# pculbertson/argus

Measured on AMD Instinct MI355X. Metric: train images/sec + val SE(3) geodesic err, 2x256x256 RGB, higher is better.
Workload: dtype bf16; 1 GPU; configs[1] cube_unity_data_small-shaped: fused train step, 64 samples (128 images) of 256x256 per rank, 2 cams, ResNet-50 + MLP head, bf16; batch_per_rank=64, global_batch=64, parallelism=dp1

## Files before the change

### argus_amd/csrc/conv.hip

```cpp
#include "common.h"
#include "internal.h"
#include "ktimer.h"
#include "igemm.h"
#include "lds_dma.h"

namespace argus {

template <typename T>
ARGUS_DEV u32x4 bn_relu_chunk(u32x4 v, const float* __restrict__ sc, const float* __restrict__ sh, int ch) {
  constexpr int E = Chunk<T>::E;
  float f[E];
  unpack(v, f);
#pragma unroll
  for (int j = 0; j < E; ++j) f[j] = fmaxf(fmaf(f[j], sc[ch + j], sh[ch + j]), 0.f);
  return pack(f);
}

constexpr int kProLds = 512;

template <typename T> struct ProCoef {
  float s[Chunk<T>::E], h[Chunk<T>::E];
  ARGUS_DEV void load(const float* __restrict__ sc, const float* __restrict__ sh, int ch) {
#pragma unroll
    for (int j = 0; j < Chunk<T>::E; j += 4) {
// ... 1599 lines not shown
  return dgrad_stages_prologue(d, p.f8 ? ARGUS_BF16 : dtype, p) ? 1 : 0;
}

static int dgrad_bn_impl(const argus_conv_desc& d, int dtype, const void* dy, const void* wt, void* dm,
                         const void* addend, const argus_bn_bwd_epilogue* bn, const argus_bn_bwd_prologue* pro,
                         bool x8, hipStream_t st) {
  if (int e = check_desc(d)) return e;
  const bool f8 = dtype == ARGUS_FP8;
  if (f8) dtype = ARGUS_BF16;
  if (d.stem) { set_error("conv_dgrad_bn: the stem input has no gradient"); return ARGUS_ERR_ARG; }
  static const argus_bn_bwd_epilogue no_epilogue = {};
  const bool epi = bn != nullptr;
  if (!epi) bn = &no_epilogue;
  const bool yrec = epi && bn->y_x;
  if (yrec && (dtype != ARGUS_BF16 || bn->y || !bn->y_w || bn->mask_mode != 3 || bn->y_k <= 0 || bn->y_k % 64)) {
    set_error("conv_dgrad_bn: y recompute needs bf16, mask mode 3, y == NULL, y_w and y_k % 64 == 0");
    return ARGUS_ERR_ARG;
  }
  if ((epi && ((!bn->y && !yrec) || !bn->mean || !bn->invstd || !bn->part || (bn->mask_mode != 2 && bn->mask_mode != 3))) ||
      (bn->mask_mode == 2 && (!bn->scale || !bn->shift || bn->y2)) || (bn->mask_mode == 3 && !bn->mask_bits) ||
      (bn->y2 && (!bn->mean2 || !bn->invstd2 || !bn->part2)) || (bn->y && bn->y == dm)) {
    set_error("conv_dgrad_bn: bad BN-backward epilogue arguments");
    return ARGUS_ERR_ARG;
  }
  if (pro && (!pro->y || !pro->ca || !pro->cb || !pro->cc || (pro->dy_out && (pro->dy_out == dy || pro->dy_out == dm)))) {
    set_error("conv_dgrad_bn: bad apply-prologue arguments");
    return ARGUS_ERR_ARG;
  }
  const Policy pol = policy_of(d);
  if (x8 && (pro || yrec || addend || (epi && bn->mask_mode != 2))) {
    set_error("conv_dgrad_bn_x8: no apply prologue, addend or y recompute; BN epilogue mask mode 2 only");
    return ARGUS_ERR_ARG;
  }
  if (!x8 && pol[kP1x1Dgrad] && epi && !yrec && bn->mask_mode == 3 && pro && !pro->dy_out && p1x1_ok(d, dtype) &&
      !(f8 && (pol[kFp8Passes] & 4)) && bn->workspace && bn->gamma && bn->ca && bn->cb && bn->cc &&
      (!bn->y2 || (bn->gamma2 && bn->ca2 && bn->cb2 && bn->cc2))) {
    dgrad_work(d, dtype, addend != nullptr, true, true, bn->y2 != nullptr);
    g_launch_bytes += 2.0 * d.n * d.ho * d.wo * d.k;
    return p1x1_launch(d, dy, wt, dm, addend, bn, pro, st);
  }
  IgParams p;
  dgrad_params(d, pol, dy, wt, dm, addend, nullptr, p);
  p.f8 = f8 && !yrec;
  if (x8) {
    int f8f, f8d;
    wp_f8_layouts(d, f8f, f8d);
    p.x8 = 1;
    p.bb.mode = epi ? 2 : 0;
    if (!f8d || !conv3x3_halo_x8_ok(p)) {
      set_error("conv_dgrad_bn_x8: not served (3x3 stride-1 halo shapes, K % 128, MX-fp8 dgrad weights: "
                "policy key 37 bit 2)");
      return ARGUS_ERR_ARG;
    }
    p.bb.mode = 0;
  }
  if (yrec) { p.bb.yx = bn->y_x; p.bb.yw = bn->y_w; p.bb.yk = bn->y_k; }
  if (pro) {
    if (!dgrad_stages_prologue(d, dtype, p)) {
      if (!pro->dy_out) {
        set_error("conv_dgrad_bn: this dgrad cannot stage the apply prologue; dy_out is required");
        return ARGUS_ERR_ARG;
      }
      if (int e = argus_bn_bwd_apply(dtype, (int64_t)d.n * d.ho * d.wo, d.k, dy, 0, nullptr, pro->y, nullptr,
                                     nullptr, pro->ca, pro->cb, pro->cc, pro->dy_out, nullptr, nullptr, nullptr,
                                     nullptr, nullptr, nullptr, st))
        return e;
      p.a = pro->dy_out;
    } else {
      p.ap.y = pro->y; p.ap.ca = pro->ca; p.ap.cb = pro->cb; p.ap.cc = pro->cc; p.ap.out = pro->dy_out;
    }
  }
// ... 301 lines not shown
```

### argus_amd/csrc/conv_p1x1.hip

```cpp
#include "common.h"
#include "igemm.h"
#include "internal.h"
#include "ktimer.h"

namespace argus {

namespace {
constexpr int kP1BM = 64, kP1BN = 128, kP1LDC = kP1BN + 8;

template <int KC> ARGUS_DEV int p1_pos(int row, int chunk) {
  return row * KC + (chunk ^ (KC >= 16 ? (row & 15) : ((row >> 1) & 7)));
}
}

struct P1Params {
  const bf16* dm;
  const bf16* ay;
  const float *ca, *cb, *cc;
  const bf16* wd;
  const bf16* addend;
  bf16* out;
  BnBwdEpi bb;
  BnFin fin;
  int P, N, G, NB, tiles;
};

template <int K, int BW>
__global__ __launch_bounds__(256, K >= 256 ? 1 : 2) void p1x1_dgrad_kernel(const P1Params p) {
  constexpr bool DUAL = BW == 4;
  constexpr int KC = K / 8;
  constexpr int ARP = 256 / KC;
  constexpr int APS = kP1BM / ARP;
  constexpr int W_B = kP1BN * K * 2, A_B = kP1BM * K * 2, C_B = kP1BM * kP1LDC * 2;
  constexpr int RED_B = 8 * 16 * 16 * 8;
  static_assert(C_B >= RED_B && A_B + C_B >= 256 * 32, "scratch");
  __shared__ __attribute__((aligned(16))) u32x4 lds[(W_B + A_B + C_B) / 16];
  __shared__ int fin_flag;
  u32x4* Wl = lds;
  u32x4* Al = lds + W_B / 16;
  bf16* Cs = reinterpret_cast<bf16*>(lds + (W_B + A_B) / 16);

  const int total = p.G * p.NB;
  const int wid = xcd_remap(blockIdx.x, total);
  const int nb = wid % p.NB, g0 = wid / p.NB;
  const int tid = threadIdx.x, lane = tid & 63, wave = tid >> 6;
  const int wm = wave >> 1, wn = wave & 1;
  const int g = lane >> 4, i16 = lane & 15;

#pragma unroll
  for (int i = 0; i < kP1BN * KC / 256; ++i) {
    const int idx = tid + 256 * i, r = idx / KC, c = idx - r * KC;
    Wl[p1_pos<KC>(r, c)] = ld16(p.wd + (size_t)(nb * kP1BN + r) * K + c * 8);
  }
  const int ac = tid % KC, ar0 = tid / KC;
  float ca[8], cb[8], cc[8];
  BwdEpiAcc<bf16, 3>::ld(ca, p.ca + ac * 8);
  BwdEpiAcc<bf16, 3>::ld(cb, p.cb + ac * 8);
  BwdEpiAcc<bf16, 3>::ld(cc, p.cc + ac * 8);
  const int ec = tid % 16, rg = tid / 16;
  const int col = nb * kP1BN + ec * 8;
  BwdEpiAcc<bf16, BW> bwd;
  bwd.init(p.bb, col);

  struct APre { u32x4 dm[APS], y[APS]; };
  struct EPre { u32x4 add[4], y[4], y2[DUAL ? 4 : 1]; unsigned bits[4]; };
  auto load_a = [&](int t, APre& S) {
#pragma unroll
    for (int i = 0; i < APS; ++i) {
      const int m = min(t * kP1BM + ar0 + ARP * i, p.P - 1);
      S.dm[i] = ld16(p.dm + (size_t)m * K + ac * 8);
      S.y[i] = ld16(p.ay + (size_t)m * K + ac * 8);
    }
  };
  auto load_e = [&](int t, EPre& S) {
#pragma unroll
    for (int i = 0; i < 4; ++i) {
      const size_t off = (size_t)min(t * kP1BM + rg + 16 * i, p.P - 1) * p.N + col;
      if (p.addend) S.add[i] = ld16(p.addend + off);
      S.y[i] = ld16(reinterpret_cast<const bf16*>(p.bb.y) + off);
      if constexpr (DUAL) S.y2[i] = ld16(reinterpret_cast<const bf16*>(p.bb.y2) + off);
      S.bits[i] = p.bb.bits[off / 8];
    }
  };

  APre A;
  EPre Ep;
  int t = g0;
  if (t < p.tiles) {
    load_a(t, A);
    load_e(t, Ep);
  }
  __syncthreads();
  for (; t < p.tiles; t += p.G) {
#pragma unroll
    for (int i = 0; i < APS; ++i) {
      const int r = ar0 + ARP * i;
      float d[8], yv[8];
      unpack(A.dm[i], d);
      unpack(A.y[i], yv);
#pragma unroll
      for (int j = 0; j < 8; ++j) d[j] = fmaf(ca[j], d[j], fmaf(cb[j], yv[j], cc[j]));
      Al[p1_pos<KC>(r, ac)] = sel(t * kP1BM + r < p.P, pack(d));
    }
    const int tn = t + p.G;
    if (tn < p.tiles) load_a(tn, A);
    __syncthreads();

    f32x4 acc[2][4];
#pragma unroll
    for (int mi = 0; mi < 2; ++mi)
#pragma unroll
      for (int ni = 0; ni < 4; ++ni) acc[mi][ni] = f32x4{0.f, 0.f, 0.f, 0.f};
#pragma unroll
    for (int kk = 0; kk < K / 32; ++kk) {
      const int ch = 4 * kk + g;
      u32x4 fa[2], fb[4];
#pragma unroll
      for (int mi = 0; mi < 2; ++mi) fa[mi] = Al[p1_pos<KC>(32 * wm + 16 * mi + i16, ch)];
#pragma unroll
      for (int ni = 0; ni < 4; ++ni) fb[ni] = Wl[p1_pos<KC>(64 * wn + 16 * ni + i16, ch)];
#pragma unroll
      for (int mi = 0; mi < 2; ++mi)
#pragma unroll
        for (int ni = 0; ni < 4; ++ni) Mma<bf16>::run(acc[mi][ni], fa[mi], fb[ni]);
    }
#pragma unroll
    for (int mi = 0; mi < 2; ++mi)
#pragma unroll
      for (int ni = 0; ni < 4; ++ni)
#pragma unroll
        for (int r = 0; r < 4; ++r)
          Cs[(32 * wm + 16 * mi + 4 * g + r) * kP1LDC + 64 * wn + 16 * ni + i16] = (bf16)acc[mi][ni][r];
    __syncthreads();

#pragma unroll
    for (int i = 0; i < 4; ++i) {
      const int r = rg + 16 * i;
      const int m = t * kP1BM + r;
      if (m >= p.P) continue;
      u32x4 v = *reinterpret_cast<const u32x4*>(Cs + r * kP1LDC + ec * 8);
      if (p.addend) {
        float f[8], o[8];
        unpack(v, f);
        unpack(Ep.add[i], o);
#pragma unroll
        for (int j = 0; j < 8; ++j) f[j] += o[j];
        v = pack(f);
      }
      st16_nt(p.out + (size_t)m * p.N + col, bwd.step(v, Ep.y[i], DUAL ? Ep.y2[DUAL ? i : 0] : Ep.y[i], Ep.bits[i]));
    }
    if (tn < p.tiles) load_e(tn, Ep);
  }
  __syncthreads();
  bwd.template reduce<kP1BN, 256>(p.bb, reinterpret_cast<float2*>(Cs), rg, 16, ec, (size_t)g0, p.N, nb * kP1BN);
  if (p.fin.mode) {
    __syncthreads();
    bn_fin_arrive<256, kP1BN>(p.fin, g0, nb, reinterpret_cast<double2*>(Al), &fin_flag);
  }
}


static int p1_occ(int K) { return K >= 256 ? 1 : 2; }

bool p1x1_ok(const argus_conv_desc& d, int dtype) {
  return dtype == ARGUS_BF16 && !d.stem && d.r == 1 && d.s == 1 && d.stride == 1 && d.pad == 0 &&
         (d.k == 64 || d.k == 128 || d.k == 256) && d.c % kP1BN == 0 && d.h == d.ho && d.w == d.wo &&
         (long)d.n * d.h * d.w > 0;
}

int p1x1_rows(const argus_conv_desc& d) {
  const int tiles = (int)(((long)d.n * d.h * d.w + kP1BM - 1) / kP1BM);
  const int nb = d.c / kP1BN;
  int G = p1_occ(d.k) * 256 / nb;
  if (G < 1) G = 1;
  return G < tiles ? G : tiles;
}

int p1x1_launch(const argus_conv_desc& d, const void* dm, const void* wd, void* out, const void* addend,
                const argus_bn_bwd_epilogue* bn, const argus_bn_bwd_prologue* pro, hipStream_t st) {
  P1Params p{};
  p.dm = reinterpret_cast<const bf16*>(dm);
  p.ay = reinterpret_cast<const bf16*>(pro->y);
  p.ca = pro->ca; p.cb = pro->cb; p.cc = pro->cc;
  p.wd = reinterpret_cast<const bf16*>(wd);
  p.addend = reinterpret_cast<const bf16*>(addend);
  p.out = reinterpret_cast<bf16*>(out);
  p.P = d.n * d.h * d.w;
  p.N = d.c;
  p.NB = d.c / kP1BN;
  p.tiles = (p.P + kP1BM - 1) / kP1BM;
  p.G = p1x1_rows(d);
  BnBwdEpi& b = p.bb;
  b.y = bn->y; b.mean = bn->mean; b.invstd = bn->invstd; b.bits = bn->mask_bits; b.y2 = bn->y2;
  b.mean2 = bn->mean2; b.invstd2 = bn->invstd2;
  b.part = reinterpret_cast<float2*>(bn->part); b.part2 = reinterpret_cast<float2*>(bn->part2);
  b.mode = 3; b.prow = p.G;
  if (bn->workspace) {
    BnFin& f = p.fin;
    f.mode = 2; f.C = d.c; f.count = (long long)p.P;
    f.cnt = reinterpret_cast<unsigned*>(bn->workspace);
    f.red = reinterpret_cast<double2*>(reinterpret_cast<char*>(bn->workspace) + kBnCounterBytes);
    f.part = reinterpret_cast<const float2*>(bn->part); f.part2 = reinterpret_cast<const float2*>(bn->part2);
    f.gamma = bn->gamma; f.bmean = bn->mean; f.binvstd = bn->invstd;
    f.dgamma = bn->dgamma; f.dbeta = bn->dbeta; f.ca = bn->ca; f.cb = bn->cb; f.cc = bn->cc;
    f.gamma2 = bn->gamma2; f.bmean2 = bn->mean2; f.binvstd2 = bn->invstd2;
    f.dgamma2 = bn->dgamma2; f.dbeta2 = bn->dbeta2; f.ca2 = bn->ca2; f.cb2 = bn->cb2; f.cc2 = bn->cc2;
    bn_fin_plan(f, p.G, 1);
    f.rows = f.T;
  }
  const dim3 grid(p.G * p.NB);
  const bool dual = bn->y2 != nullptr;
  static const char* names[3][2] = {{"argus::p1x1_dgrad_kernel<64, 3>", "argus::p1x1_dgrad_kernel<64, 4>"},
                                    {"argus::p1x1_dgrad_kernel<128, 3>", "argus::p1x1_dgrad_kernel<128, 4>"},
                                    {"argus::p1x1_dgrad_kernel<256, 3>", "argus::p1x1_dgrad_kernel<256, 4>"}};
  const int ki = d.k == 64 ? 0 : (d.k == 128 ? 1 : 2);
  const char* nm = names[ki][dual];
  if (d.k == 64) {
    if (dual) timed_launch(nm, p1x1_dgrad_kernel<64, 4>, grid, dim3(256), st, p);
    else timed_launch(nm, p1x1_dgrad_kernel<64, 3>, grid, dim3(256), st, p);
  } else if (d.k == 128) {
    if (dual) timed_launch(nm, p1x1_dgrad_kernel<128, 4>, grid, dim3(256), st, p);
    else timed_launch(nm, p1x1_dgrad_kernel<128, 3>, grid, dim3(256), st, p);
  } else {
    if (dual) timed_launch(nm, p1x1_dgrad_kernel<256, 4>, grid, dim3(256), st, p);
    else timed_launch(nm, p1x1_dgrad_kernel<256, 3>, grid, dim3(256), st, p);
  }
  return check_launch("p1x1_dgrad_kernel");
}

struct P1FParams {
  const bf16* x;
  const bf16* w;
  float2* part;
  int* counts;
  int P, N, G, NB, tiles;
  BnFwdFin ffin;
};

template <int K, int BNC>
__global__ __launch_bounds__(256) void p1x1_fwd_stats_kernel(const P1FParams p) {
  constexpr int KC = K / 8;
  constexpr int ARP = 256 / KC;
  constexpr int APS = kP1BM / ARP;
  constexpr int NI = BNC / 32;
  constexpr int DEPTH = K <= 256 ? 2 : 1;
  constexpr int W_B = BNC * K * 2, A_B = kP1BM * K * 2;
  static_assert(A_B >= 2 * BNC * 16, "reduction scratch");
  __shared__ __attribute__((aligned(16))) u32x4 lds[(W_B + A_B) / 16];
  u32x4* Wl = lds;
  u32x4* Al = lds + W_B / 16;

  const int total = p.G * p.NB;
  const int wid = xcd_remap(blockIdx.x, total);
  const int nb = wid % p.NB, g0 = wid / p.NB;
  const int tid = threadIdx.x, lane = tid & 63, wave = tid >> 6;
  const int wm = wave >> 1, wn = wave & 1;
  const int g = lane >> 4, i16 = lane & 15;

// ... 205 lines not shown
```

### argus_amd/engine.py

```python
from __future__ import annotations

import ctypes as C
import contextlib
from dataclasses import dataclass

import torch

from argus_amd._lib import BnFwdFin, BF16, F32, FP8, BnBwdEpilogue, BnBwdPrologue, ConvDesc, lib, ptr, stream


@dataclass(frozen=True)
class Block:
    prefix: str
    cin: int
    width: int
    cout: int
    stride: int
    has_ds: bool


def resnet50_blocks() -> list[Block]:
    blocks, inplanes = [], 64
    for L, (planes, n, stride) in enumerate([(64, 3, 1), (128, 4, 2), (256, 6, 2), (512, 3, 2)], start=1):
        for i in range(n):
# ... 35 lines not shown
        self.rdim = resnet_output_dim
        self.dtype = dtype
        low = dtype in ("bf16", "fp8")
        self.dt = BF16 if low else F32
        self.cdt = FP8 if dtype == "fp8" else self.dt
        self.tdt = torch.bfloat16 if low else torch.float32
        self.E = 8 if low else 4
        self.materialize = low
        self.device = torch.device(device)
        self.blocks = resnet50_blocks()
        self.shape = None
        self.saved = False
        self.debug: dict | None = None
        self.wgrad_overlap = True
        self.fuse_apply = True
        self.wgrad_apply = True
        self.fold_fin = True
        self.fold_fwd_fin = False
        self.fold_stem_fin = True
        self._side: torch.cuda.Stream | None = None
        self._pending: dict = {}
        self._last_side = None
        self.side_batch = True
        self._deferred: list = []
        self._side_seq = 0
        self._waited_seq = 0
        self._stem_overlap = True
        self.tail_main = True
        self._tail: list = []
        self.dy_ring = 12
        self.side_priority = 0
        self.fuse_dgw = True
        self.fuse_out = True
        self.yrec_epi = False
        self.y3_free = False
        self.x8 = True
        self.a2_in_stats = False

    def _t(self, *shape, dtype=None):
        return torch.empty(shape, dtype=dtype or self.tdt, device=self.device)

    def _f(self, *shape):
        return torch.empty(shape, dtype=torch.float32, device=self.device)

    def ensure(self, B: int, H: int, W: int) -> None:
        if self.shape == (B, H, W):
            return
        self.shape = (B, H, W)
        N = B * self.n_cams
        self.N = N
        L = self.L
        dt = self.dt
        convs: dict[str, _Conv] = {}

        def add(name, n, h, w, c, k, ks, s, p, stem=False):
            d = ConvDesc(n, h, w, c, k, ks, ks, s, p, _out(h, ks, s, p), _out(w, ks, s, p), int(stem)).with_tuning(
                self.tuning)
            if stem:
                wf = self._t(k, 256)
                wd = None
            else:
                wf = self._t(k, ks * ks * c)
                wd = self._t(c, ks * ks * k)
            rows = L.dll.argus_conv_fwd_stat_rows(C.byref(d), self.cdt)
            tile = L.dll.argus_conv_fwd_stat_tile(C.byref(d), dt)
            fl = C.c_int64(0)
            tags = tuple(L.dll.argus_conv_launch_info(C.byref(d), dt, ps, C.byref(fl)) for ps in range(3))
            so = (L.dll.argus_conv_fwd_stats_only_rows(C.byref(d), BF16),
                  L.dll.argus_conv_fwd_stats_only_tile(C.byref(d), BF16))
            pb = max(L.dll.argus_conv_fwd_stat_part_bytes(C.byref(d), self.cdt, 0),
                     L.dll.argus_conv_fwd_stat_part_bytes(C.byref(d), dt, 0),
                     L.dll.argus_conv_fwd_stat_part_bytes(C.byref(d), BF16, 1))
            convs[name] = _Conv(name, d, wf, wd, rows, tile, tags, fl.value, *so, part_bytes=pb)
            return d.ho, d.wo

        H1, W1 = add("resnet.conv1", N, H, W, 3, 64, 7, 2, 3, stem=True)
        H2, W2 = _out(H1, 3, 2, 1), _out(W1, 3, 2, 1)
        self.stem_hw = (H1, W1)
        self.pool_hw = (H2, W2)
        self.x0 = self._t(N, H, W, 4)
        self.y0 = self._t(N, H1, W1, 64)
        self.p0 = self._t(N, H2, W2, 64)
        self.amax = torch.empty((N, H2, W2, 64), dtype=torch.uint8, device=self.device)
        act = []
        h, w = H2, W2
        max_elems = N * H1 * W1 * 64
        for b in self.blocks:
            add(b.prefix + ".conv1", N, h, w, b.cin, b.width, 1, 1, 0)
            ho, wo = add(b.prefix + ".conv2", N, h, w, b.width, b.width, 3, b.stride, 1)
            add(b.prefix + ".conv3", N, ho, wo, b.width, b.cout, 1, 1, 0)
            if b.has_ds:
                add(b.prefix + ".downsample.0", N, h, w, b.cin, b.cout, 1, b.stride, 0)
            a = {
                "hw_in": (h, w), "hw": (ho, wo),
                "y1": self._t(N, h, w, b.width), "y2": self._t(N, ho, wo, b.width),
                "y3": self._t(N, ho, wo, b.cout), "out": self._t(N, ho, wo, b.cout),
                "yd": self._t(N, ho, wo, b.cout) if b.has_ds else None,
                "a1": self._t(N, h, w, b.width) if self.materialize else None,
                "a2": self._t(N, ho, wo, b.width) if self.materialize else None,
                "bits": torch.empty(N * ho * wo * b.cout // self.E, dtype=torch.uint8, device=self.device),
            }
            max_elems = max(max_elems, N * h * w * b.cin, N * h * w * b.width, N * ho * wo * b.cout)
            act.append(a)
            h, w = ho, wo
        self.act = act
        self.final_hw = (h, w)
        self.convs = convs
        self.x8_conv = {}
        x8_bytes = 16
        for b in self.blocks:
            n = b.prefix + ".conv2"
            d_ = convs[n].desc
            on = self.x8 and self.cdt == FP8 and self.materialize
            f = on and bool(L.dll.argus_conv_x8_ok(C.byref(d_), 0))
            g = on and bool(L.dll.argus_conv_x8_ok(C.byref(d_), 1))
            self.x8_conv[n] = (f, g)
            if f:
                x8_bytes = max(x8_bytes, d_.n * d_.h * d_.w * d_.c * 33 // 32)
            if g:
                x8_bytes = max(x8_bytes, d_.n * d_.ho * d_.wo * d_.k * 33 // 32)
        self.x8buf = torch.empty(x8_bytes, dtype=torch.uint8, device=self.device)

        self.bn_names = ["resnet.bn1"]
        for b in self.blocks:
            self.bn_names += [b.prefix + ".bn1", b.prefix + ".bn2", b.prefix + ".bn3"]
            if b.has_ds:
                self.bn_names.append(b.prefix + ".downsample.1")
        chans = {"resnet.bn1": 64}
        for b in self.blocks:
# ... 15 lines not shown
        for b, a in zip(self.blocks, act):
            for hw, c in ((a["hw_in"], b.width), (a["hw"], b.width), (a["hw"], b.cout)):
                px = N * hw[0] * hw[1]
                max_bwd = max(max_bwd, L.dll.argus_bn_bwd_rows(px, c) * c)
        max_bwd = max(max_bwd, L.dll.argus_bn_bwd_rows(N * H1 * W1, 64) * 64,
                      L.dll.argus_maxpool_bwd_bn_rows(dt, N, H1, W1, 64) * 64)
        for cv in convs.values():
            if not cv.desc.stem:
                d_ = cv.desc
                max_bwd = max(max_bwd, L.dll.argus_conv_dgrad_bn_rows(C.byref(d_), self.cdt) * d_.c,
                              (4 - (-(d_.n * d_.h * d_.w) // 64)) * d_.c)
        f8_1x1 = (self.tuning or {}).get(37, L.dll.argus_conv_policy_default(37)) & 4
        self.dgw_dt = BF16 if self.cdt == FP8 and not f8_1x1 else self.cdt
        self.dgw = {n for n, cv in convs.items() if self.fuse_dgw and n.endswith((".conv3", ".downsample.0"))
                    and not cv.desc.stem and L.dll.argus_conv_dgrad_wgrad_ok(C.byref(cv.desc), self.dgw_dt)}
        dgws = 16
        for n in self.dgw:
            d_ = C.byref(convs[n].desc)
            max_bwd = max(max_bwd, L.dll.argus_conv_dgrad_wgrad_bn_rows(d_, self.dgw_dt) * convs[n].desc.c)
            dgws = max(dgws, L.dll.argus_conv_dgrad_wgrad_workspace_bytes(d_, self.dgw_dt))
        self.dgw_ws = torch.empty(dgws, dtype=torch.uint8, device=self.device)
        self.bwd_part = self._f(max_bwd * 2)
        self.bwd_part2 = self._f(max_bwd * 2)
        ws = max(L.dll.argus_conv_wgrad_workspace_bytes(C.byref(cv.desc), dt) for cv in convs.values())
        self.wg_ws = torch.empty(ws, dtype=torch.uint8, device=self.device)
        self.wg_ws_bytes = ws
        wss = L.dll.argus_conv_wgrad_workspace_bytes(C.byref(convs["resnet.conv1"].desc), dt)
        ds0 = self.blocks[0].prefix + ".downsample.0"
        if ds0 in convs:
            wss = max(wss, L.dll.argus_conv_wgrad_workspace_bytes(C.byref(convs[ds0].desc), dt))
        self.wg_ws_stem = torch.empty(wss, dtype=torch.uint8, device=self.device)
        self.stages_pro = {n: bool(L.dll.argus_conv_dgrad_stages_prologue(C.byref(cv.desc), self.cdt))
                           for n, cv in convs.items() if not cv.desc.stem}
        self.gbuf = [self._t(max_elems) for _ in range(3)]
        nring = max(8, self.dy_ring)
        self.dyring = [self._t(max_elems) for _ in range(nring)]
        self._ring_i = 0

        Fd = 512 * 4
        self.feat = self._f(N, Fd)
        self.h0 = self._f(N, self.rdim)
        self.g0 = self._f(B, self.n_cams * self.rdim)
        self.h1, self.g1 = self._f(B, 128), self._f(B, 128)
        self.h2, self.g2 = self._f(B, 128), self._f(B, 128)
        self.pred = self._f(B, 6)
        self.dh2, self.dh1 = self._f(B, 128), self._f(B, 128)
        self.dh0 = self._f(B, self.n_cams * self.rdim)
        self.dfeat = self._f(N, Fd)
        D = self.n_cams * self.rdim
        shapes = [(N, self.rdim, Fd), (B, 128, D), (B, 128, 128), (B, 6, 128), (6, 128, B), (B, 128, 6),
                  (128, 128, B), (128, D, B), (B, D, 128), (self.rdim, Fd, N), (N, Fd, self.rdim)]
        hws = max(L.dll.argus_gemm_f32_workspace_bytes(*sh) for sh in shapes)
        self.gemm_ws = torch.empty(max(hws, 16), dtype=torch.uint8, device=self.device)
        self.gemm_ws_side = torch.empty(max(hws, 16), dtype=torch.uint8, device=self.device)

    def _bn_train(self, P, Bf, name, rows, tile, count, part=None, ws=None):
        st = self.bn_state[name]
        mom = Bf.get(name + ".momentum", 0.1)
        part = self.stat_part if part is None else part
        ws = self.bn_ws if ws is None else ws
        self.L.bn_finalize(self.bn_ch[name], rows, tile, ptr(part), count, ptr(P[name + ".weight"]),
                           ptr(P[name + ".bias"]), C.c_float(Bf.get(name + ".eps", 1e-5)), C.c_float(mom),
                           ptr(Bf[name + ".running_mean"]), ptr(Bf[name + ".running_var"]),
                           ptr(Bf[name + ".num_batches_tracked"]), ptr(st[0]), ptr(st[1]), ptr(st[2]), ptr(st[3]),
                           ptr(ws), stream())

# ... 63 lines not shown
            return
        self.L.bn_apply(self.dt, px, ch, ptr(y), ptr(st[2]), ptr(st[3]), None, None, None, 1, ptr(out), None, stream())

    def prepare_weights(self, P) -> None:
        ws = []
        for name in self.convs:
            w = P[name + ".weight"]
            if w.dtype != torch.float32 or w.device != self.device:
                raise TypeError(f"{name}.weight must be fp32 on {self.device}")
            ws.append(w)
        key = tuple((w.data_ptr(), w.stride(), cv.wf.data_ptr(), cv.wd.data_ptr() if cv.wd is not None else 0)
                    for w, cv in zip(ws, self.convs.values()))
        if getattr(self, "_wp_key", None) != key:
            cvs = list(self.convs.values())
            n = len(cvs)
            descs = (ConvDesc * n)(*[cv.desc for cv in cvs])
            masters = (C.c_void_p * n)(*[w.data_ptr() for w in ws])
            strides = (C.c_int64 * (4 * n))(*[x for w in ws for x in w.stride()])
            wfs = (C.c_void_p * n)(*[cv.wf.data_ptr() for cv in cvs])
            wds = (C.c_void_p * n)(*[cv.wd.data_ptr() if cv.wd is not None else None for cv in cvs])
            nbytes = self.L.dll.argus_conv_weight_prep_table_bytes(n)
            host = (C.c_uint8 * nbytes)()
            nblk = C.c_int(0)
            self.L.conv_weight_prep_table(n, descs, masters, strides, wfs, wds, host, nbytes, C.byref(nblk))
            self._wp_table = torch.frombuffer(bytearray(host), dtype=torch.uint8).to(self.device)
            self._wp_n, self._wp_blocks, self._wp_key = n, nblk.value, key
        self.L.conv_weight_prep_batch(self.cdt, self._wp_n, ptr(self._wp_table), self._wp_blocks, stream())

    def forward(self, x: torch.Tensor, P: dict, Bf: dict, training: bool) -> torch.Tensor:
        B, Cn, H, W = x.shape
        if Cn != 3 * self.n_cams:
            raise ValueError(f"expected {3 * self.n_cams} input channels, got {Cn}")
        self.ensure(B, H, W)
        x = x.contiguous()
        L, dt, s = self.L, self.dt, stream()
        N = self.N
        self.prepare_weights(P)
        if x.dtype == torch.uint8:
            L.images_u8_to_nhwc4(dt, N, H, W, ptr(x), ptr(self.x0), s)
        else:
            if x.dtype != torch.float32:
                x = x.float()
            L.images_to_nhwc4(dt, N, H, W, ptr(x), ptr(self.x0), s)
        self._conv_bn(P, Bf, "resnet.conv1", "resnet.bn1", self.x0, self.y0, None, training)
        st = self.bn_state["resnet.bn1"]
        H1, W1 = self.stem_hw
        L.maxpool_fwd(dt, N, H1, W1, 64, ptr(self.y0), ptr(st[2]), ptr(st[3]), ptr(self.p0), ptr(self.amax), s)
        h = self.p0
        for bi, (b, a) in enumerate(zip(self.blocks, self.act)):
            pf = b.prefix
            ds_done = None
            if b.has_ds and self.wgrad_overlap:
                ds_done = self._on_side(lambda: self._conv_bn(P, Bf, pf + ".downsample.0", pf + ".downsample.1", h,
                                                              a["yd"], None, training, self.stat_part_ds,
                                                              self.bn_ws_ds))
            self._conv_bn(P, Bf, pf + ".conv1", pf + ".bn1", h, a["y1"], None, training)
            tail = self._fused_tail()
            if self.materialize:
                x8f = self.x8_conv[pf + ".conv2"][0]
                self._act(pf + ".bn1", a["y1"], a["a1"], N * a["hw_in"][0] * a["hw_in"][1], b.width,
                          self.x8buf if x8f else None)
                self._conv_bn(P, Bf, pf + ".conv2", pf + ".bn2", a["a1"], a["y2"], None, training,
                              x8=self.x8buf if x8f else None)
                if tail and training and self.a2_in_stats:
                    self._conv_bn(P, Bf, pf + ".conv3", pf + ".bn3", a["y2"], None, pf + ".bn2", training,
                                  x_out=a["a2"])
# ... 114 lines not shown
                if dbg is not None:
                    dbg[key + "." + pf] = t[:n].view(*shape).clone()

            cap("b_dout", dh, px_o * b.cout, (N, ho, wo, b.cout))
            fuse = self.fuse_apply
            dza, dzb = g[1], g[2]
            if rows3 is None:
                L.bn_bwd_reduce(dt, px_o, b.cout, ptr(dh), 3, ptr(a["bits"]), ptr(a["y3"]), None, None,
                                ptr(self.bn_state[pf + ".bn3"][0]), ptr(self.bn_state[pf + ".bn3"][1]),
                                ptr(self.bwd_part), None, None, None, None, s)
                rows3 = L.dll.argus_bn_bwd_rows(px_o, b.cout)
                self._bn_bwd_fin(P, G, pf + ".bn3", px_o, b.cout, self.bwd_part, rows3)
                cf, st3 = self.bn_coef[pf + ".bn3"], self.bn_state[pf + ".bn3"]
                self._guard(dy3)
                L.bn_bwd_apply(dt, px_o, b.cout, ptr(dh), 3, ptr(a["bits"]), ptr(a["y3"]), None, None, ptr(cf[0]),
                               ptr(cf[1]), ptr(cf[2]), ptr(dy3), ptr(dh), None, None, None, None, None, s)
                pro3 = None
            else:
                if rows3:
                    self._bn_bwd_fin(P, G, pf + ".bn3", px_o, b.cout, self.bwd_part, rows3)
                    if b.has_ds:
                        self._bn_bwd_fin(P, G, pf + ".downsample.1", px_o, b.cout, self.bwd_part2, rows3)
                if fuse:
                    pro3 = (pf + ".bn3", a["y3"], dy3)
                    if b.has_ds and idx == 0 and (not ds_dgw or dbg is not None):
                        self._bn_apply_bwd(pf + ".downsample.1", px_o, b.cout, dh, a["yd"], dyd)
                else:
                    pro3 = None
                    self._bn_apply_bwd(pf + ".bn3", px_o, b.cout, dh, a["y3"], dy3,
                                       (pf + ".downsample.1", a["yd"], dyd) if b.has_ds else None)
            dgw = wg3_apply and self.fold_fin and pf + ".conv3" in self.dgw
            if dgw:
                r2 = self._dgrad_wgrad_bn(pf + ".conv3", dh, dza, pf + ".bn2", a["y2"], pf + ".bn3",
                                          None if self._y3_free(idx) else a["y3"], a["a2"], P, G)
                if dy3 is not None:
                    self._bn_apply_bwd(pf + ".bn3", px_o, b.cout, dh, a["y3"], dy3)
            else:
                r2 = self._dgrad_bn(pf + ".conv3", dh if pro3 else dy3, dza, None, pf + ".bn2", a["y2"], 2, P=P, G=G,
                                    pro=pro3)
            if dy3 is not None:
                cap("b_dy3", dy3, px_o * b.cout, (N, ho, wo, b.cout))
            cap("b_dz2", dza, px_o * b.width, (N, ho, wo, b.width))
            s2 = self.bn_state[pf + ".bn2"]
            if dgw:
                pass
            elif wg3_apply:
                self._wgrad_apply(pf + ".conv3", a["a2"], dh, pf + ".bn3", a["y3"], G)
            elif a["a2"] is not None:
                self._wgrad(pf + ".conv3", a["a2"], None, dy3, G)
            else:
                self._wgrad(pf + ".conv3", a["y2"], s2, dy3, G)
            if r2:
                self._bn_bwd_fin(P, G, pf + ".bn2", px_o, b.width, self.bwd_part, r2)
            dy2 = self._next_dy()
            x8d = self.x8_conv[pf + ".conv2"][1]
            if fuse and not x8d:
                pro2 = (pf + ".bn2", a["y2"], dy2)
            else:
                pro2 = None
                self._bn_apply_bwd(pf + ".bn2", px_o, b.width, dza, a["y2"], dy2, dy8=self.x8buf if x8d else None)
            if wg1_apply:
                dzb = self._next_dy()
            r1 = self._dgrad_bn(pf + ".conv2", dza if pro2 else dy2, dzb, None, pf + ".bn1", a["y1"], 2, P=P, G=G,
                                pro=pro2, x8=self.x8buf if x8d else None)
            cap("b_dy2", dy2, px_o * b.width, (N, ho, wo, b.width))
            cap("b_dz1", dzb, px_i * b.width, (N, hi, wi, b.width))
            s1 = self.bn_state[pf + ".bn1"]
            if self.materialize:
                self._wgrad(pf + ".conv2", a["a1"], None, dy2, G)
            else:
                self._wgrad(pf + ".conv2", a["y1"], s1, dy2, G)
            if r1:
                self._bn_bwd_fin(P, G, pf + ".bn1", px_i, b.width, self.bwd_part, r1)
            dy1 = None if wg1_apply and dbg is None else self._next_dy()
            pro1 = None
            if fuse and idx > 0:
                pro1 = (pf + ".bn1", a["y1"], None if wg1_apply else dy1)
            else:
                self._bn_apply_bwd(pf + ".bn1", px_i, b.width, dzb, a["y1"], dy1)
            dx = self._next_dy()
            c1_in = dzb if pro1 else dy1
            if idx > 0:
                pb, pa = self.blocks[idx - 1], self.act[idx - 1]
                second = (pb.prefix + ".downsample.1", pa["yd"]) if pb.has_ds else None
                yrec = self._yrec(pb, pa)
                y3p = None if yrec else pa["y3"]
                if b.has_ds:
                    self._dgrad_plain_or_pro(pf + ".conv1", c1_in, dx, pro1)
                    rows3 = self._dgrad_bn(pf + ".downsample.0", dh if fuse else dyd, dx, dx, pb.prefix + ".bn3",
                                           y3p, 3, pa["bits"], second, P=P, G=G,
                                           pro=(pf + ".downsample.1", a["yd"], dyd) if fuse else None, yrec=yrec)
                else:
                    rows3 = self._dgrad_bn(pf + ".conv1", c1_in, dx, dh, pb.prefix + ".bn3", y3p, 3, pa["bits"],
                                           second, P=P, G=G, pro=pro1, yrec=yrec)
            else:
                self._dgrad(pf + ".conv1", dy1, dx)
                if ds_dgw:
                    self._dgrad_wgrad_bn(pf + ".downsample.0", dh, dx, None, None, pf + ".downsample.1", a["yd"],
                                         h_in, P, G, addend=dx)
                elif b.has_ds:
                    self._dgrad(pf + ".downsample.0", dyd, dx, addend=dx)
            if dy1 is not None:
                if pro1 is not None and pro1[2] is None:
                    self._bn_apply_bwd(pf + ".bn1", px_i, b.width, dzb, a["y1"], dy1)
                cap("b_dy1", dy1, px_i * b.width, (N, hi, wi, b.width))
            if b.has_ds:
                cap("b_dyd", dyd, px_o * b.cout, (N, ho, wo, b.cout))
            if wg1_apply:
                self._wgrad_apply(pf + ".conv1", h_in, dzb, pf + ".bn1", a["y1"], G)
            else:
                self._wgrad(pf + ".conv1", h_in, None, dy1, G)
            if b.has_ds and not ds_dgw:
                if (idx == 0 and on_ready is None and self.tail_main and self.wgrad_overlap and self._stem_overlap
                        and self.fuse_apply):
                    cvd = self.convs[pf + ".downsample.0"]
                    self._tail.append((cvd, lambda cvd=cvd, x=h_in, dy=dyd: self.L.conv_wgrad(
                        C.byref(cvd.desc), self.dt, ptr(x), None, None, ptr(dy), ptr(G[pf + ".downsample.0.weight"]),
                        ptr(self.wg_ws_stem), self.wg_ws_stem.numel(), stream())))
# ... 21 lines not shown
                self._bn_bwd_fin(P, G, "resnet.bn1", N * H1 * W1, 64, self.bwd_part,
                                 L.dll.argus_maxpool_bwd_bn_rows(dt, N, H1, W1, 64))
            cv = self.convs["resnet.conv1"]
            ap = BnBwdPrologue(ptr(self.y0), ptr(cf[0]), ptr(cf[1]), ptr(cf[2]), None)
            fn = lambda: L.conv_wgrad_apply(C.byref(cv.desc), dt, ptr(self.x0), ptr(dz0), C.byref(ap),
                                            ptr(G["resnet.conv1.weight"]), ptr(self.wg_ws_stem),
                                            self.wg_ws_stem.numel(), stream())
            if not self._stem_overlap:
                self._join()
            self._launch(cv, 2, fn)
            for cvt, fnt in self._tail:
                self._launch(cvt, 2, fnt)
            self._tail.clear()
            if dx_img is not None:
                self._stem_dgrad(dz0, ap, dx_img)
        else:
            L.maxpool_bwd(dt, N, H1, W1, 64, ptr(dh), ptr(self.amax), ptr(dz0), s)
            self._bn_bwd(P, G, "resnet.bn1", N * H1 * W1, 64, dz0, 2, None, self.y0, dy0, None)
            self._wgrad("resnet.conv1", self.x0, None, dy0, G)
            if dx_img is not None:
                self._stem_dgrad(dy0, None, dx_img)
        self._join()
        if on_ready is not None:
            on_ready("resnet.conv1.weight", self._comm)

    def _stem_dgrad(self, dy, ap, dx) -> None:
        cv = self.convs["resnet.conv1"]
        self._launch(cv, 1, lambda: self.L.conv_stem_dgrad(C.byref(cv.desc), self.dt, ptr(dy), ptr(cv.wf),
                                                            C.byref(ap) if ap is not None else None, ptr(dx),
                                                            stream()))
        if self.debug is not None:
            self.debug["bwd.dx"] = dx.clone()

    def _y3_free(self, idx: int) -> bool:
        b = self.blocks[idx]
        c3 = b.prefix + ".conv3"
        return (self.y3_free and self._fused_tail() and self.debug is None and idx < len(self.blocks) - 1
                and self.fuse_apply and self.wgrad_apply and self.fold_fin and c3 in self.dgw
                and self.stages_pro[c3] and self._yrec(b, self.act[idx]) is not None)

    def _yrec(self, blk, act):
        if not (self.yrec_epi and self.materialize and act["a2"] is not None):
            return None
        if self.cdt == FP8 and (self.tuning or {}).get(37, self.L.dll.argus_conv_policy_default(37)) & 4:
            return None
        return act["a2"], self.convs[blk.prefix + ".conv3"].wf, blk.width

    def _dgrad_bn(self, conv, dy, dm, addend, bn, y, mode, bits=None, second=None, P=None, G=None, pro=None,
                  yrec=None, x8=None):
        cv = self.convs[conv]
        st = self.bn_state[bn]
        e = BnBwdEpilogue()
        if self.fold_fin:
            cf = self.bn_coef[bn]
            e.workspace, e.gamma, e.dgamma, e.dbeta = ptr(self.bn_ws), ptr(P[bn + ".weight"]), ptr(G[bn + ".weight"]), \
                ptr(G[bn + ".bias"])
            e.ca, e.cb, e.cc = ptr(cf[0]), ptr(cf[1]), ptr(cf[2])
            if second is not None:
                cf2 = self.bn_coef[second[0]]
                e.gamma2, e.dgamma2, e.dbeta2 = ptr(P[second[0] + ".weight"]), ptr(G[second[0] + ".weight"]), \
                    ptr(G[second[0] + ".bias"])
                e.ca2, e.cb2, e.cc2 = ptr(cf2[0]), ptr(cf2[1]), ptr(cf2[2])
        e.y, e.mean, e.invstd, e.mask_mode = ptr(y), ptr(st[0]), ptr(st[1]), mode
        if yrec is not None:
            e.y_x, e.y_w, e.y_k = ptr(yrec[0]), ptr(yrec[1]), yrec[2]
        if mode == 2:
            e.scale, e.shift = ptr(st[2]), ptr(st[3])
        else:
            e.mask_bits = ptr(bits)
        e.part = ptr(self.bwd_part)
        if second is not None:
            st2 = self.bn_state[second[0]]
            e.y2, e.mean2, e.invstd2, e.part2 = ptr(second[1]), ptr(st2[0]), ptr(st2[1]), ptr(self.bwd_part2)
        pp = self._prologue(pro)
        self._guard(dm)
        if x8 is not None:
            self._launch(cv, 1, lambda: self.L.conv_dgrad_bn_x8(C.byref(cv.desc), ptr(x8), ptr(cv.wd), ptr(dm),
# ... 188 lines not shown
```

Measured before the change: 9680 images/s.

## Recompute bn3 output inside persistent 1x1 dgrad kernel for 64-wide blocks

Adds a YR variant of the persistent 1x1 dgrad+BN-backward kernel. It recomputes the conv3 pre-BN output y3 from a2 and the conv3 weights with an extra MFMA pass in LDS instead of reading a stored y3 tensor. The engine turns y3 recompute and y3-free mode on by default for width-64 blocks not followed by a downsample, and skips allocating y3 for those blocks. This trades extra matmul work and LDS use (which may cut occupancy) for less HBM traffic and memory in the backward pass.

Result: faster. 9784 images/s, median of 6 (+1.1%).

```diff
diff --git a/argus_amd/csrc/conv.hip b/argus_amd/csrc/conv.hip
--- a/argus_amd/csrc/conv.hip
+++ b/argus_amd/csrc/conv.hip
@@ -1655,11 +1655,16 @@
     set_error("conv_dgrad_bn_x8: no apply prologue, addend or y recompute; BN epilogue mask mode 2 only");
     return ARGUS_ERR_ARG;
   }
-  if (!x8 && pol[kP1x1Dgrad] && epi && !yrec && bn->mask_mode == 3 && pro && !pro->dy_out && p1x1_ok(d, dtype) &&
+  if (!x8 && pol[kP1x1Dgrad] && epi && (!yrec || (bn->y_k == 64 && d.k == 64)) && bn->mask_mode == 3 && pro &&
+      !pro->dy_out && p1x1_ok(d, dtype) &&
       !(f8 && (pol[kFp8Passes] & 4)) && bn->workspace && bn->gamma && bn->ca && bn->cb && bn->cc &&
       (!bn->y2 || (bn->gamma2 && bn->ca2 && bn->cb2 && bn->cc2))) {
     dgrad_work(d, dtype, addend != nullptr, true, true, bn->y2 != nullptr);
     g_launch_bytes += 2.0 * d.n * d.ho * d.wo * d.k;
+    if (yrec) {
+      g_launch_bytes -= 2.0 * (double)d.n * d.h * d.w * (d.c - bn->y_k);
+      g_launch_work += 2.0 * d.n * d.h * d.w * d.c * bn->y_k;
+    }
     return p1x1_launch(d, dy, wt, dm, addend, bn, pro, st);
   }
   IgParams p;
diff --git a/argus_amd/csrc/conv_p1x1.hip b/argus_amd/csrc/conv_p1x1.hip
--- a/argus_amd/csrc/conv_p1x1.hip
+++ b/argus_amd/csrc/conv_p1x1.hip
@@ -11,6 +11,8 @@
 template <int KC> ARGUS_DEV int p1_pos(int row, int chunk) {
   return row * KC + (chunk ^ (KC >= 16 ? (row & 15) : ((row >> 1) & 7)));
 }
+
+ARGUS_DEV int p1_ypos(int row, int chunk) { return row * 16 + (chunk ^ (((row >> 2) & 3) << 1)); }
 }
 
 struct P1Params {
@@ -25,20 +27,27 @@
   int P, N, G, NB, tiles;
 };
 
-template <int K, int BW>
+template <int K, int BW, bool YR>
 __global__ __launch_bounds__(256, K >= 256 ? 1 : 2) void p1x1_dgrad_kernel(const P1Params p) {
+  static_assert(!YR || K == 64, "the recompute is built for the 64-wide blocks (two workgroups per CU)");
   constexpr bool DUAL = BW == 4;
+  constexpr int K2 = 64, KC2 = K2 / 8;
   constexpr int KC = K / 8;
   constexpr int ARP = 256 / KC;
   constexpr int APS = kP1BM / ARP;
   constexpr int W_B = kP1BN * K * 2, A_B = kP1BM * K * 2, C_B = kP1BM * kP1LDC * 2;
   constexpr int RED_B = 8 * 16 * 16 * 8;
+  constexpr int W3_B = YR ? kP1BN * K2 * 2 : 0, X_B = YR ? kP1BM * K2 * 2 : 0;
   static_assert(C_B >= RED_B && A_B + C_B >= 256 * 32, "scratch");
-  __shared__ __attribute__((aligned(16))) u32x4 lds[(W_B + A_B + C_B) / 16];
+  static_assert(!YR || A_B + X_B >= kP1BM * kP1BN * 2, "the y tile reuses the A / yx tiles");
+  __shared__ __attribute__((aligned(16))) u32x4 lds[(W_B + W3_B + A_B + X_B + C_B) / 16];
   __shared__ int fin_flag;
   u32x4* Wl = lds;
-  u32x4* Al = lds + W_B / 16;
-  bf16* Cs = reinterpret_cast<bf16*>(lds + (W_B + A_B) / 16);
+  u32x4* W3l = lds + W_B / 16;
+  u32x4* Al = lds + (W_B + W3_B) / 16;
+  u32x4* Xl = Al + A_B / 16;
+  bf16* Cs = reinterpret_cast<bf16*>(Xl + X_B / 16);
+  u32x4* Yl = Al;
 
   const int total = p.G * p.NB;
   const int wid = xcd_remap(blockIdx.x, total);
@@ -51,6 +60,13 @@
   for (int i = 0; i < kP1BN * KC / 256; ++i) {
     const int idx = tid + 256 * i, r = idx / KC, c = idx - r * KC;
     Wl[p1_pos<KC>(r, c)] = ld16(p.wd + (size_t)(nb * kP1BN + r) * K + c * 8);
+  }
+  if constexpr (YR) {
+#pragma unroll
+    for (int i = 0; i < kP1BN * KC2 / 256; ++i) {
+      const int idx = tid + 256 * i, r = idx / KC2, c = idx - r * KC2;
+      W3l[p1_pos<KC2>(r, c)] = ld16(reinterpret_cast<const bf16*>(p.bb.yw) + (size_t)(nb * kP1BN + r) * K2 + c * 8);
+    }
   }
   const int ac = tid % KC, ar0 = tid / KC;
   float ca[8], cb[8], cc[8];
@@ -62,14 +78,15 @@
   BwdEpiAcc<bf16, BW> bwd;
   bwd.init(p.bb, col);
 
-  struct APre { u32x4 dm[APS], y[APS]; };
-  struct EPre { u32x4 add[4], y[4], y2[DUAL ? 4 : 1]; unsigned bits[4]; };
+  struct APre { u32x4 dm[APS], y[APS], x[YR ? APS : 1]; };
+  struct EPre { u32x4 add[4], y[YR ? 1 : 4], y2[DUAL ? 4 : 1]; unsigned bits[4]; };
   auto load_a = [&](int t, APre& S) {
 #pragma unroll
     for (int i = 0; i < APS; ++i) {
       const int m = min(t * kP1BM + ar0 + ARP * i, p.P - 1);
       S.dm[i] = ld16(p.dm + (size_t)m * K + ac * 8);
       S.y[i] = ld16(p.ay + (size_t)m * K + ac * 8);
+      if constexpr (YR) S.x[i] = ld16(reinterpret_cast<const bf16*>(p.bb.yx) + (size_t)m * K2 + ac * 8);
     }
   };
   auto load_e = [&](int t, EPre& S) {
@@ -77,7 +94,7 @@
     for (int i = 0; i < 4; ++i) {
       const size_t off = (size_t)min(t * kP1BM + rg + 16 * i, p.P - 1) * p.N + col;
       if (p.addend) S.add[i] = ld16(p.addend + off);
-      S.y[i] = ld16(reinterpret_cast<const bf16*>(p.bb.y) + off);
+      if constexpr (!YR) S.y[i] = ld16(reinterpret_cast<const bf16*>(p.bb.y) + off);
       if constexpr (DUAL) S.y2[i] = ld16(reinterpret_cast<const bf16*>(p.bb.y2) + off);
       S.bits[i] = p.bb.bits[off / 8];
     }
@@ -101,6 +118,7 @@
 #pragma unroll
       for (int j = 0; j < 8; ++j) d[j] = fmaf(ca[j], d[j], fmaf(cb[j], yv[j], cc[j]));
       Al[p1_pos<KC>(r, ac)] = sel(t * kP1BM + r < p.P, pack(d));
+      if constexpr (YR) Xl[p1_pos<KC2>(r, ac)] = A.x[i];
     }
     const int tn = t + p.G;
     if (tn < p.tiles) load_a(tn, A);
@@ -131,6 +149,36 @@
 #pragma unroll
         for (int r = 0; r < 4; ++r)
           Cs[(32 * wm + 16 * mi + 4 * g + r) * kP1LDC + 64 * wn + 16 * ni + i16] = (bf16)acc[mi][ni][r];
+    if constexpr (YR) {
+#pragma unroll
+      for (int mi = 0; mi < 2; ++mi)
+#pragma unroll
+        for (int ni = 0; ni < 4; ++ni) acc[mi][ni] = f32x4{0.f, 0.f, 0.f, 0.f};
+#pragma unroll
+      for (int s2 = 0; s2 < K2 / 32; ++s2) {
+        const int ch = 4 * s2 + g;
+        u32x4 fa[2], fb[4];
+#pragma unroll
+        for (int mi = 0; mi < 2; ++mi) fa[mi] = Xl[p1_pos<KC2>(32 * wm + 16 * mi + i16, ch)];
+#pragma unroll
+        for (int ni = 0; ni < 4; ++ni) fb[ni] = W3l[p1_pos<KC2>(64 * wn + 16 * ni + i16, ch)];
+#pragma unroll
+        for (int mi = 0; mi < 2; ++mi)
+#pragma unroll
+          for (int ni = 0; ni < 4; ++ni) Mma<bf16>::run(acc[mi][ni], fa[mi], fb[ni]);
+      }
+      __syncthreads();
+      bf16* Ys = reinterpret_cast<bf16*>(Yl);
+#pragma unroll
+      for (int mi = 0; mi < 2; ++mi)
+#pragma unroll
+        for (int ni = 0; ni < 4; ++ni)
+#pragma unroll
+          for (int r = 0; r < 4; ++r) {
+            const int cl = 64 * wn + 16 * ni + i16;
+            Ys[p1_ypos(32 * wm + 16 * mi + 4 * g + r, cl >> 3) * 8 + (cl & 7)] = (bf16)acc[mi][ni][r];
+          }
+    }
     __syncthreads();
 
 #pragma unroll
@@ -147,9 +195,13 @@
         for (int j = 0; j < 8; ++j) f[j] += o[j];
         v = pack(f);
       }
-      st16_nt(p.out + (size_t)m * p.N + col, bwd.step(v, Ep.y[i], DUAL ? Ep.y2[DUAL ? i : 0] : Ep.y[i], Ep.bits[i]));
+      u32x4 yv;
+      if constexpr (YR) yv = Yl[p1_ypos(r, ec)];
+      else yv = Ep.y[i];
+      st16_nt(p.out + (size_t)m * p.N + col, bwd.step(v, yv, DUAL ? Ep.y2[DUAL ? i : 0] : yv, Ep.bits[i]));
     }
     if (tn < p.tiles) load_e(tn, Ep);
+    if constexpr (YR) __syncthreads();
   }
   __syncthreads();
   bwd.template reduce<kP1BN, 256>(p.bb, reinterpret_cast<float2*>(Cs), rg, 16, ec, (size_t)g0, p.N, nb * kP1BN);
@@ -191,6 +243,8 @@
   p.tiles = (p.P + kP1BM - 1) / kP1BM;
   p.G = p1x1_rows(d);
   BnBwdEpi& b = p.bb;
+  const bool yr = bn->y_x != nullptr;
+  b.yx = bn->y_x; b.yw = bn->y_w; b.yk = bn->y_k;
   b.y = bn->y; b.mean = bn->mean; b.invstd = bn->invstd; b.bits = bn->mask_bits; b.y2 = bn->y2;
   b.mean2 = bn->mean2; b.invstd2 = bn->invstd2;
   b.part = reinterpret_cast<float2*>(bn->part); b.part2 = reinterpret_cast<float2*>(bn->part2);
@@ -215,15 +269,18 @@
                                     {"argus::p1x1_dgrad_kernel<256, 3>", "argus::p1x1_dgrad_kernel<256, 4>"}};
   const int ki = d.k == 64 ? 0 : (d.k == 128 ? 1 : 2);
   const char* nm = names[ki][dual];
-  if (d.k == 64) {
-    if (dual) timed_launch(nm, p1x1_dgrad_kernel<64, 4>, grid, dim3(256), st, p);
-    else timed_launch(nm, p1x1_dgrad_kernel<64, 3>, grid, dim3(256), st, p);
+  if (yr) {
+    if (dual) timed_launch("argus::p1x1_dgrad_kernel<64, 4, true>", p1x1_dgrad_kernel<64, 4, true>, grid, dim3(256), st, p);
+    else timed_launch("argus::p1x1_dgrad_kernel<64, 3, true>", p1x1_dgrad_kernel<64, 3, true>, grid, dim3(256), st, p);
+  } else if (d.k == 64) {
+    if (dual) timed_launch(nm, p1x1_dgrad_kernel<64, 4, false>, grid, dim3(256), st, p);
+    else timed_launch(nm, p1x1_dgrad_kernel<64, 3, false>, grid, dim3(256), st, p);
   } else if (d.k == 128) {
-    if (dual) timed_launch(nm, p1x1_dgrad_kernel<128, 4>, grid, dim3(256), st, p);
-    else timed_launch(nm, p1x1_dgrad_kernel<128, 3>, grid, dim3(256), st, p);
+    if (dual) timed_launch(nm, p1x1_dgrad_kernel<128, 4, false>, grid, dim3(256), st, p);
+    else timed_launch(nm, p1x1_dgrad_kernel<128, 3, false>, grid, dim3(256), st, p);
   } else {
-    if (dual) timed_launch(nm, p1x1_dgrad_kernel<256, 4>, grid, dim3(256), st, p);
-    else timed_launch(nm, p1x1_dgrad_kernel<256, 3>, grid, dim3(256), st, p);
+    if (dual) timed_launch(nm, p1x1_dgrad_kernel<256, 4, false>, grid, dim3(256), st, p);
+    else timed_launch(nm, p1x1_dgrad_kernel<256, 3, false>, grid, dim3(256), st, p);
   }
   return check_launch("p1x1_dgrad_kernel");
 }
diff --git a/argus_amd/engine.py b/argus_amd/engine.py
--- a/argus_amd/engine.py
+++ b/argus_amd/engine.py
@@ -91,8 +91,8 @@
         self.side_priority = 0
         self.fuse_dgw = True
         self.fuse_out = True
-        self.yrec_epi = False
-        self.y3_free = False
+        self.yrec_epi = "persistent"
+        self.y3_free = True
         self.x8 = True
         self.a2_in_stats = False
 
@@ -153,7 +153,7 @@
             a = {
                 "hw_in": (h, w), "hw": (ho, wo),
                 "y1": self._t(N, h, w, b.width), "y2": self._t(N, ho, wo, b.width),
-                "y3": self._t(N, ho, wo, b.cout), "out": self._t(N, ho, wo, b.cout),
+                "y3": None, "out": self._t(N, ho, wo, b.cout),
                 "yd": self._t(N, ho, wo, b.cout) if b.has_ds else None,
                 "a1": self._t(N, h, w, b.width) if self.materialize else None,
                 "a2": self._t(N, ho, wo, b.width) if self.materialize else None,
@@ -235,6 +235,7 @@
         self.wg_ws_stem = torch.empty(wss, dtype=torch.uint8, device=self.device)
         self.stages_pro = {n: bool(L.dll.argus_conv_dgrad_stages_prologue(C.byref(cv.desc), self.cdt))
                            for n, cv in convs.items() if not cv.desc.stem}
+        self._alloc_y3()
         self.gbuf = [self._t(max_elems) for _ in range(3)]
         nring = max(8, self.dy_ring)
         self.dyring = [self._t(max_elems) for _ in range(nring)]
@@ -364,6 +365,7 @@
         if Cn != 3 * self.n_cams:
             raise ValueError(f"expected {3 * self.n_cams} input channels, got {Cn}")
         self.ensure(B, H, W)
+        self._alloc_y3()
         x = x.contiguous()
         L, dt, s = self.L, self.dt, stream()
         N = self.N
@@ -544,7 +546,7 @@
             dgw = wg3_apply and self.fold_fin and pf + ".conv3" in self.dgw
             if dgw:
                 r2 = self._dgrad_wgrad_bn(pf + ".conv3", dh, dza, pf + ".bn2", a["y2"], pf + ".bn3",
-                                          None if self._y3_free(idx) else a["y3"], a["a2"], P, G)
+                                          None if self._y3_recomputed(idx) else a["y3"], a["a2"], P, G)
                 if dy3 is not None:
                     self._bn_apply_bwd(pf + ".bn3", px_o, b.cout, dh, a["y3"], dy3)
             else:
@@ -595,7 +597,7 @@
             if idx > 0:
                 pb, pa = self.blocks[idx - 1], self.act[idx - 1]
                 second = (pb.prefix + ".downsample.1", pa["yd"]) if pb.has_ds else None
-                yrec = self._yrec(pb, pa)
+                yrec = self._yrec(idx - 1)
                 y3p = None if yrec else pa["y3"]
                 if b.has_ds:
                     self._dgrad_plain_or_pro(pf + ".conv1", c1_in, dx, pro1)
@@ -683,17 +685,28 @@
         if self.debug is not None:
             self.debug["bwd.dx"] = dx.clone()
 
+    def _y3_recomputed(self, idx: int) -> bool:
+        c3 = self.blocks[idx].prefix + ".conv3"
+        return (self.y3_free and self._fused_tail() and idx < len(self.blocks) - 1
+                and self.fuse_apply and self.wgrad_apply and self.fold_fin and c3 in self.dgw
+                and self.stages_pro[c3] and self._yrec(idx) is not None)
+
     def _y3_free(self, idx: int) -> bool:
-        b = self.blocks[idx]
-        c3 = b.prefix + ".conv3"
-        return (self.y3_free and self._fused_tail() and self.debug is None and idx < len(self.blocks) - 1
-                and self.fuse_apply and self.wgrad_apply and self.fold_fin and c3 in self.dgw
-                and self.stages_pro[c3] and self._yrec(b, self.act[idx]) is not None)
-
-    def _yrec(self, blk, act):
+        return self.debug is None and self._y3_recomputed(idx)
+
+    def _alloc_y3(self) -> None:
+        N = self.N
+        for idx, (b, a) in enumerate(zip(self.blocks, self.act)):
+            if a["y3"] is None and not self._y3_free(idx):
+                a["y3"] = self._t(N, *a["hw"], b.cout)
+
+    def _yrec(self, idx: int):
+        blk, act = self.blocks[idx], self.act[idx]
         if not (self.yrec_epi and self.materialize and act["a2"] is not None):
             return None
         if self.cdt == FP8 and (self.tuning or {}).get(37, self.L.dll.argus_conv_policy_default(37)) & 4:
+            return None
+        if self.yrec_epi == "persistent" and (blk.width != 64 or self.blocks[idx + 1].has_ds):
             return None
         return act["a2"], self.convs[blk.prefix + ".conv3"].wf, blk.width
 
```
